# huawei-noah/Speech-Backbones

Hardware: NVIDIA H100
Metric: mel-frames/sec at N=50 reverse-diffusion steps (higher is better)
Workload: dtype f32

## Files before the change

speech-backbones_b200/csrc/sbk_api.cu:

```cuda
#include "sbk_host.h"

#include <math.h>
#include <stdarg.h>
#include <stdio.h>
#include <stdlib.h>
#include <string.h>

#include <algorithm>
#include <map>
#include <string>
#include <vector>

using namespace sbk;

static thread_local char g_err[1024] = "";
int sbk::fail(int code, const char* fmt, ...) {
    va_list ap;
    va_start(ap, fmt);
    vsnprintf(g_err, sizeof(g_err), fmt, ap);
    va_end(ap);
    return code;
}

namespace {
// ... 323 lines not shown
        CU(cudaMemcpy(h->d_freqs, f.data(), half * sizeof(float), cudaMemcpyHostToDevice));
    }
    if (!h->d_zero) {
        CU(cudaMalloc(&h->d_zero, 8192));
        CU(cudaMemset(h->d_zero, 0, 8192));
    }
    free_plan(h);
    h->is_packed = true;
    return SBK_OK;
}

namespace {
struct Bufs {
    float *A[3], *Bf[3], *X[3], *Y[3], *S[3], *D[3], *U1;
    float *kv_part, *ctx, *w_eff, *b_eff;
    std::map<const void*, float*> lo;
};
}

static size_t layout(const sbk_handle* h, int B, int T, int tb_rows, Arena& ar, Bufs* bf, Plan* pl) {
    const sbk_config& c = h->cfg;
    const int dim = c.dim, H = c.n_feats;
    const size_t P[3] = {(size_t)H * T, (size_t)(H / 2) * (T / 2), (size_t)(H / 4) * (T / 4)};
    const int C[3] = {dim, dim * 2, dim * 4};
    auto f = [&](size_t n) { return (float*)ar.take(n * sizeof(float)); };
    const size_t osz = c.precision == SBK_PREC_BF16 ? 2 : 4;
    const bool x3 = c.precision == SBK_PREC_FP32X3;
    Bufs b{};
    auto fo = [&](size_t n) {
        float* r = (float*)ar.take(n * osz);
        if (x3) { float* l = (float*)ar.take(n * osz); if (r) b.lo[r] = l; }
        return r;
    };
    for (int l = 0; l < 3; ++l) {
        const size_t n = (size_t)B * P[l] * C[l];
        b.A[l] = f(n); b.Bf[l] = fo(n); b.X[l] = fo(n); b.Y[l] = fo(n);
        b.S[l] = l > 0 ? fo(n) : nullptr;
        b.D[l] = l > 0 ? fo((size_t)B * P[l] * C[l - 1]) : nullptr;
    }
    b.U1 = fo((size_t)B * P[1] * C[1]);
    const size_t mt0 = (P[0] + attn_kv_tile_pixels() - 1) / attn_kv_tile_pixels();
    b.kv_part = f((size_t)B * mt0 * kHeads * kKvPartFloats);
    b.ctx = f((size_t)B * kHeads * 1024);
    b.w_eff = f((size_t)B * C[2] * C[2] * (x3 ? 2 : 1));
    b.b_eff = f(C[2]);
    if (bf) *bf = b;
    Plan dummy;
    Plan& p = pl ? *pl : dummy;
// ... 48 lines not shown
    auto stats_slot = [&]() { return pl.stats + (size_t)(gn_slot++) * B * kGroups * 2; };
    auto gnref = [&](const double* st, const std::string& blk, int C, int lvl) {
        GnRef g; g.stats = st; g.gamma = h->w.get(blk + ".block.1.weight"); g.beta = h->w.get(blk + ".block.1.bias");
        g.inv_count = 1.0f / ((float)(C / kGroups) * (float)Hs[lvl] * (float)Ws[lvl]);
        return g;
    };
    auto base_ig = [&](int geom, int lvl_in, int lvl_out) {
        IgemmParams p; memset(&p, 0, sizeof(p));
        p.geom = geom; p.B = B; p.T = T;
        p.Hin = Hs[lvl_in]; p.Win = Ws[lvl_in]; p.Hout = Hs[lvl_out]; p.Wout = Ws[lvl_out];
        p.in_lvl = lvl_in; p.out_lvl = lvl_out; p.mask = pl.mask; p.step = pl.step_cur;
        return p;
    };
    const bool use_tc = c.precision != SBK_PREC_FP32;
    const bool x3 = c.precision == SBK_PREC_FP32X3;
    auto LO = [&](const void* q) -> float* { auto it = bf.lo.find(q); return it == bf.lo.end() ? nullptr : it->second; };
    const int num_sms = device_sm_count();
    const char* rows_env = getenv("SBK_CONV3_ROWS");
    const int conv_rows_env = rows_env ? atoi(rows_env) : 0;
    const bool b16 = c.precision == SBK_PREC_BF16;
    const double osz = b16 ? 2.0 : 4.0;
    const int fmt_raw = use_tc ? 1 : 0, fmt_opnd = b16 ? 2 : fmt_raw;
    const int form = b16 ? FORM_BF16 : (x3 ? FORM_X3 : (use_tc ? FORM_TF32 : FORM_NHWC));
    auto push = [&](Op& op, const float* dbg, int64_t numel) {
        op.dbg_ptr = dbg; op.dbg_numel = numel;
        const bool raw_out = op.kind == OP_FIRST || op.kind == OP_CTX || (op.kind == OP_CONVTC && op.tc.geom == G_C3);
        op.dbg_fmt = raw_out ? fmt_raw : fmt_opnd;
        if (op.kind == OP_IGEMM) {
            const IgemmParams& p = op.ig;
            const double cin = p.c0 + p.c1, opx = (double)B * p.Hout * p.Wout, ipx = (double)B * p.Hin * p.Win;
            const double taps = p.geom == G_PW ? 1 : (p.geom == G_UP ? 4 : 9);
// ... 9 lines not shown
            op.bytes = 4.0 * B * H0 * T * (op.fn.C + 3.0);
        }
        pl.ops.push_back(op);
    };
    auto npix = [&](int lvl) { return (int64_t)B * Hs[lvl] * Ws[lvl]; };

    auto tc_conv = [&](const std::string& name, int geom, const std::string& wkey, const std::string& bkey, int lvl,
                       const float* in0, int c0, const float* in1, int c1, int cout, float* out, double* st) {
        Op op; op.name = name; op.kind = OP_CONVTC;
        ConvTcParams& p = op.tc; memset(&p, 0, sizeof(p));
        p.geom = geom; p.in0 = in0; p.c0 = c0; p.in1 = in1; p.c1 = c1; p.H = Hs[lvl]; p.W = Ws[lvl]; p.B = B;
        p.Ho = p.H; p.Wo = p.W;
        p.wpk = h->w.get(wkey); p.bias = bkey.empty() ? nullptr : h->w.get(bkey); p.out = out; p.Cout = cout;
        p.epi = EPI_PLAIN; p.ostats = st; p.mask = pl.mask; p.T = T; p.lvl = lvl; p.zero_page = h->d_zero;
        p.form = form; p.nt = conv_tc_ntile(geom, cout, form);
        if (x3) { p.in0_lo = LO(in0); p.in1_lo = LO(in1); p.out_corr = geom != G_C3 ? LO(out) : nullptr; }
        if (geom == G_C3) {
            const long long wt = (Ws[lvl] + 127) / 128;
            const long long tiles2 = (long long)B * wt * ((Hs[lvl] + 1) / 2) * (cout / 64);
            bool two = tiles2 >= 4LL * num_sms;
            if (conv_rows_env == 1 || conv_rows_env == 2) two = conv_rows_env == 2;
            const bool wide = p.nt == 128;
            if (two && (!wide || h->w.packed.count(wkey + "64"))) {
                p.rows = 2;
                if (wide) { p.nt = 64; p.wpk = h->w.get(wkey + "64"); }
            } else if (wide) {
                const long long tiles = (long long)B * wt * Hs[lvl] * (cout / 128);
                if (tiles * 2 <= num_sms && h->w.packed.count(wkey + "64")) { p.nt = 64; p.wpk = h->w.get(wkey + "64"); }
            }
        }
        const double taps = geom == G_PW ? 1.0 : (geom == G_UP ? 4.0 : 9.0);
// ... 29 lines not shown
            Op op = tc_conv(r.prefix + ".block1.raw", G_C3, r.prefix + ".block1.wtc", r.prefix + ".block1.block.0.bias", lvl,
                            in0, c0, in1, c1, r.cout, A, st1);
            push(op, A, npix(lvl) * r.cout);
        } else {
            ffma_block_conv(r.prefix + ".block1.raw", r.prefix + ".block1.w", r.prefix + ".block1.block.0.bias", lvl,
                            in0, c0, in1, c1, r.cout, A, st1, PRO_MASK, nullptr, k);
        }
        const GnRef g1 = gnref(st1, r.prefix + ".block1", r.cout, lvl);
        float* h2 = Bb;
        if (use_tc) {
            {
                Op op; op.kind = OP_GNACT; op.name = r.prefix + ".block1.act";
                GnActParams& p = op.ga; memset(&p, 0, sizeof(p));
                p.raw = A; p.gn = g1; p.tb = pl.tb + h->tb_off[k]; p.tb_stride = pl.tb_stride; p.step = pl.step_cur;
                p.mask = pl.mask; p.T = T; p.lvl = lvl; p.out = Bb; p.B = B; p.H = Hs[lvl]; p.W = Ws[lvl]; p.C = r.cout;
                p.form = form; p.out_lo = LO(Bb);
                op.bytes = (4.0 + osz) * npix(lvl) * r.cout;
                push(op, nullptr, 0);
            }
            Op op = tc_conv(r.prefix + ".block2.raw", G_C3, r.prefix + ".block2.wtc", r.prefix + ".block2.block.0.bias", lvl,
                            Bb, r.cout, nullptr, 0, r.cout, A, st2);
            push(op, A, npix(lvl) * r.cout);
            h2 = A;
        } else {
            ffma_block_conv(r.prefix + ".block2.raw", r.prefix + ".block2.w", r.prefix + ".block2.block.0.bias", lvl,
                            A, r.cout, nullptr, 0, r.cout, Bb, st2, PRO_GN, &g1, k);
        }
        const GnRef g2 = gnref(st2, r.prefix + ".block2", r.cout, lvl);
        if (k == 0 || r.cin == r.cout) {
            Op op; op.kind = OP_RESFINAL; op.name = r.prefix + ".out";
            ResFinalParams& p = op.rf; memset(&p, 0, sizeof(p));
            p.h2raw = h2; p.gn = g2;
            p.mask = pl.mask; p.T = T; p.lvl = lvl; p.out = out; p.B = B; p.H = Hs[lvl]; p.W = Ws[lvl]; p.C = r.cout;
            p.out_mask = store_masked ? 1 : 0; p.form = form; p.out_lo = LO(out);
            if (k == 0) {
                p.x = nullptr; p.mu = pl.mu; p.xt = pl.xt; p.spk_s = pl.spk_s; p.cin = cin0;
                p.wres = h->w.get(r.prefix + ".res.w"); p.bres = h->w.get(r.prefix + ".res_conv.bias");
                if (vc) { p.r_extra = pl.vc_rextra; p.step = pl.step_cur; }
                pl.first_res_op = (int)pl.ops.size();
            } else {
                p.x = in0;
            }
            op.bytes = (4.0 + (k == 0 ? 0.0 : osz) + osz) * npix(lvl) * r.cout;
            push(op, out, npix(lvl) * r.cout);
        } else if (use_tc) {
            Op op = tc_conv(r.prefix + ".out", G_PW, r.prefix + ".res.wtc", r.prefix + ".res_conv.bias", lvl,
                            in0, c0, in1, c1, r.cout, out, nullptr);
            op.tc.epi = EPI_RES; op.tc.rraw = h2; op.tc.rgn = g2; op.tc.out_mask = store_masked ? 1 : 0;
            op.bytes += 4.0 * npix(lvl) * r.cout;
// ... 3 lines not shown
            op.ig = base_ig(G_PW, lvl, lvl);
            IgemmParams& p = op.ig;
            p.in0 = in0; p.c0 = c0; p.in1 = in1; p.c1 = c1;
            p.w = h->w.get(r.prefix + ".res.w"); p.bias = h->w.get(r.prefix + ".res_conv.bias");
            p.out = out; p.Cout = r.cout; p.pro = PRO_MASK; p.epi = EPI_RES;
            p.rraw = h2; p.rgn = g2;
            push(op, out, npix(lvl) * r.cout);
        }
    };
    auto attention = [&](int k, int lvl, const float* x, float* out) {
        const AttnInfo& a = h->attns[k];
        int mt = igemm_mtiles(G_PW, Hs[lvl], Ws[lvl], Hs[lvl], Ws[lvl]);
        if (use_tc) {
            Op op = tc_conv(a.prefix + ".kvpart", G_PW, a.prefix + ".kv.wtc", "", lvl, x, a.c, nullptr, 0, 256, nullptr, nullptr);
            op.tc.epi = EPI_KV; op.tc.kv_part = bf.kv_part;
            op.bytes = (x3 ? 8.0 : osz) * npix(lvl) * a.c;
            op.flops += 2.0 * npix(lvl) * 4096.0;
            mt = (Hs[lvl] * Ws[lvl] + attn_kv_tile_pixels() - 1) / attn_kv_tile_pixels();
            push(op, nullptr, 0);
        } else {
            Op op; op.kind = OP_IGEMM; op.name = a.prefix + ".kvpart";
            op.ig = base_ig(G_PW, lvl, lvl);
            IgemmParams& p = op.ig;
            p.in0 = x; p.c0 = a.c; p.w = h->w.get(a.prefix + ".kv.w"); p.Cout = 256; p.pro = PRO_NONE; p.epi = EPI_KV;
            p.kv_part = bf.kv_part; p.out = nullptr;
            push(op, nullptr, 0);
        }
        {
            Op op; op.kind = OP_CTX; op.name = a.prefix + ".ctx";
            op.cx.kv_part = bf.kv_part; op.cx.mtiles = mt; op.cx.ctx = bf.ctx; op.cx.B = B;
            push(op, bf.ctx, (int64_t)B * kHeads * 1024);
// ... 674 lines not shown
```

speech-backbones_b200/csrc/sbk_attn_x3.cu:

```cuda
#include "sbk_tc.cuh"

#include <type_traits>

namespace sbk {

using namespace tc;

namespace kx3 {
constexpr int PX = 64;
constexpr int KCH = 8;
constexpr int XS = KCH * PX * 16;
constexpr int WS = 2 * KCH * 128 * 16;
constexpr int STAGE = XS + WS;
constexpr int STAGES = 2;
constexpr int OPI = (PX / 4) * 128 * 16;
constexpr int THREADS = 256 + 32;
constexpr int NBARS = 2 * STAGES;
constexpr size_t SMEM = (size_t)STAGES * STAGE + 4 * OPI + 4 * 128 * 4 + NBARS * 8 + 16;
static_assert(SMEM <= 227 * 1024, "shared memory budget");
}

template <int MODE>
__global__ void __launch_bounds__(kx3::THREADS, 1) k_attn_kv_wg(const ConvTcParams p) {
    using namespace kx3;
    constexpr bool X3 = MODE == 2;
    constexpr int EPC = MODE == 1 ? 8 : 4;
    constexpr int KMAIN = MODE == 1 ? K_BF16 : K_TF32;
    extern __shared__ __align__(1024) uint8_t smem[];
    uint8_t* sS = smem;
    uint8_t* kp = sS + STAGES * STAGE;
    uint8_t* vt = kp + OPI;
    uint8_t* pc = vt + OPI;
    uint8_t* vc = pc + OPI;
    float* s_mx = reinterpret_cast<float*>(vc + OPI);
// ... 13 lines not shown
    if (tid == 0) {
        for (int s = 0; s < STAGES; ++s) { mbar_init(full(s), 1); mbar_init(empty(s), 8); }
        fence_barrier_init();
    }
    __syncthreads();

    if (warp < 8) {
        const int wg = warp >> 2, wt = tid & 127;
        const int row = tid & 127, half = tid >> 7;
        constexpr uint32_t D_HI = desc_hi(128);
        const uint32_t s0 = smem_u32(sS);
        uint32_t it = 0;
        for (int t = blockIdx.x; t < total; t += gridDim.x) {
            const int b = t / items, mt = t - b * items;
            float acc[64];
            for (int ks = 0; ks < ksteps_t; ++ks, ++it) {
                const int s = it % STAGES;
                mbar_wait(full(s), (it / STAGES) & 1);
                const uint32_t xs = s0 + s * STAGE;
                const uint32_t x_lo = desc_lo(xs, PX * 16), w_lo = desc_lo(xs + XS + wg * (KCH * 128 * 16), 128 * 16);
                auto issue = [&](auto kind) {
#pragma unroll
                    for (int kk = 0; kk < KCH / 2; ++kk)
                        wgmma<128, decltype(kind)::value>(acc, desc_pack(x_lo + (uint32_t)(kk * 2 * PX), D_HI),
                                                          desc_pack(w_lo + (uint32_t)(kk * 2 * 128), D_HI), (ks | kk) != 0 ? 1u : 0u);
                };
                wg_fence();
                if (X3 && (ks & 1) == 0) issue(std::integral_constant<int, K_F16>{});
                else issue(std::integral_constant<int, KMAIN>{});
                wg_commit();
                wg_wait<0>();
                wg_fence_regs(acc);
                __syncwarp();
                if (lane == 0) mbar_arrive(empty(s));
            }
            {
                uint8_t* img = wg == 0 ? kp : vt;
#pragma unroll
                for (int i = 0; i < 64; ++i) {
                    const int px = frag_row(wt, i), r = frag_col(wt, i);
                    *reinterpret_cast<float*>(img + ((size_t)(px / 4) * 128 + r) * 16 + (px % 4) * 4) = acc[i];
                }
            }
            asm volatile("bar.sync 1, 256;" ::: "memory");
// ... 73 lines not shown
        }
    } else {
        uint32_t it = 0;
        const int chs = p.c0 / EPC;
        for (int t = blockIdx.x; t < total; t += gridDim.x) {
            const int b = t / items, mt = t - b * items;
            const int m0 = mt * PX, m_hi = m0 + PX < HW ? m0 + PX : HW;
            const int hh0 = m0 / p.W, ww0 = m0 - hh0 * p.W;
            for (int ks = 0; ks < ksteps_t; ++ks, ++it) {
                const int s = it % STAGES;
                const int kb = X3 ? ks >> 1 : ks;
                const bool corr = X3 && (ks & 1) == 0;
                const uint32_t xs = smem_u32(sS) + s * STAGE;
                if (lane == 0) {
                    mbar_wait(empty(s), ((it / STAGES) & 1) ^ 1);
                    mbar_arrive_expect_tx(full(s), STAGE);
                    bulk_g2s(xs + XS, reinterpret_cast<const uint8_t*>(p.wpk) + (size_t)(X3 ? 2 * kb + (corr ? 1 : 0) : ks) * WS, WS, full(s));
                }
                __syncwarp();
                if (lane < KCH) {
                    const uint8_t* src = reinterpret_cast<const uint8_t*>(corr ? p.in0_lo : p.in0);
                    const int k = lane, cl = kb * KCH + k;
                    int m = m0, hh = hh0, ww = ww0, qx = 0;
                    while (m < m_hi) {
                        const int n = (p.W - ww) < (m_hi - m) ? (p.W - ww) : (m_hi - m);
                        bulk_g2s(xs + (k * PX + qx) * 16, src + (((long long)(b * p.H + hh) * chs + cl) * p.W + ww) * 16,
                                 (uint32_t)n * 16u, full(s));
                        m += n; qx += n; ++hh; ww = 0;
                    }
                    if (qx < PX) bulk_g2s(xs + (k * PX + qx) * 16, p.zero_page, (uint32_t)(PX - qx) * 16u, full(s));
                }
            }
        }
    }
}

// ... 19 lines not shown
```

speech-backbones_b200/csrc/sbk_conv_tc.cu:

```cuda
#include "sbk_tc.cuh"

#include <cuda_fp16.h>
#include <string.h>
#include <type_traits>

namespace sbk {

namespace tc {

constexpr int TPX = 128;
constexpr int NCONS = 256;
constexpr int NTHREADS = NCONS + 128;
constexpr int PROD_REGS = 40, CONS_REGS = 232;
static_assert(128 * PROD_REGS + NCONS * CONS_REGS <= 65536, "register file");

template <int GEOM, int R = 1> struct Geo;
template <int R> struct Geo<G_C3, R> {
    static_assert(R == 1 || R == 2, "3x3 tiles are 1 or 2 rows");
    static constexpr int ROWS = R, HR = R + 2, PXP = TPX + 2, TAPS = 9, KCH = 2, NACC = R;
};
template <> struct Geo<G_PW> { static constexpr int ROWS = 1, HR = 1, PXP = TPX, TAPS = 1, KCH = 8, NACC = 1; };
template <> struct Geo<G_DOWN> { static constexpr int ROWS = 1, HR = 3, PXP = 2 * (TPX + 1), TAPS = 9, KCH = 2, NACC = 1; };
template <> struct Geo<G_UP> { static constexpr int ROWS = 1, HR = 3, PXP = TPX + 2, TAPS = 16, KCH = 2, NACC = 4; };

template <int K> struct GeoC1 { static constexpr int ROWS = 1, HR = 1, PXP = TPX + 64, TAPS = K, KCH = 2, NACC = 1; };
template <> struct Geo<G_C1K3> : GeoC1<3> {};
template <> struct Geo<G_C1K7> : GeoC1<7> {};
// ... 7 lines not shown

using namespace tc;


template <int GEOM, int NT, int R = 1> struct Depth {
    using G = Geo<GEOM, R>;
    static constexpr int STAGE_BYTES = G::KCH * G::HR * G::PXP * 16 + G::TAPS * G::KCH * NT * 16;
    static constexpr int LDS = NT + 4;
    static constexpr int SD_BYTES = TPX * LDS * 4;
    static constexpr int FIT = (220 * 1024 - SD_BYTES) / STAGE_BYTES;
    static constexpr int STAGES = FIT > 6 ? 6 : FIT;
    static constexpr size_t SMEM = (size_t)STAGES * STAGE_BYTES + SD_BYTES + 3 * STAGES * 8 + 128 * 4 * G::ROWS + 3 * NT * 4 + 64;
    static_assert(STAGES >= 2, "need at least 2 stages");
    static_assert(SMEM <= 227 * 1024, "shared memory budget");
};

template <int GEOM, bool BF16, int NT, bool RES, bool X3, bool VOC = false, int R = 1>
__device__ __forceinline__ void conv_tc_body(const ConvTcParams& p) {
    static_assert(!(X3 && BF16), "fp32x3 runs on tf32 operands");
    using G = Geo<GEOM, R>;
    using D = Depth<GEOM, NT, R>;
    constexpr int NACC = G::NACC, ROWS = G::ROWS;
    constexpr bool ROW2 = ROWS == 2;
    constexpr bool CHUNKED = X3 && GEOM != G_UP;
    const int FLUSH = CHUNKED ? 6 : (1 << 30);
    constexpr int STAGES = D::STAGES, LDS = D::LDS;
    constexpr int LAG = STAGES >= 3 ? STAGES - 2 : 0;
    constexpr int HR = G::HR, PXP = G::PXP, TAPS = G::TAPS, KCH = G::KCH;
    constexpr int EPC = BF16 ? 8 : 4;
    constexpr int CPS = KCH * EPC;
// ... 9 lines not shown
    constexpr int KMAIN = BF16 ? K_BF16 : K_TF32;

    extern __shared__ __align__(1024) uint8_t smem[];
    uint8_t* sA = smem;
    uint8_t* sB = sA + STAGES * A_STAGE_BYTES;
    float* sD = reinterpret_cast<float*>(sB + STAGES * B_STAGE_BYTES);
    uint64_t* bars = reinterpret_cast<uint64_t*>(sD + TPX * LDS);
    float* s_st = reinterpret_cast<float*>(bars + 3 * STAGES);
    float* s_rg = s_st + 128 * ROWS;

    const int tid = threadIdx.x, warp = __shfl_sync(0xffffffffu, tid >> 5, 0), lane = tid & 31;
    const int Cin = p.c0 + p.c1;
    const int HW = p.H * p.W;
    const int ksteps = Cin / CPS * conv_tc_stage_rows(GEOM);
    const int ksteps_t = X3 ? 2 * ksteps : ksteps;
    const int wt_w = (GEOM == G_DOWN ? p.Wo : p.W), wt_h = (GEOM == G_DOWN ? p.Ho : p.H);
    const int wtiles = (wt_w + SPAN - 1) / SPAN;
    const int mtiles = GEOM == G_PW ? (HW + TPX - 1) / TPX : wtiles * ((wt_h + ROWS - 1) / ROWS);
    const int ntn = p.Cout / NT;
    const int total_tiles = p.B * mtiles * ntn;
    auto decode = [&](int t, int& b, int& h0, int& w0, int& n0) {
        const int nt = t % ntn; const int r = t / ntn;
        const int mt = r % mtiles; b = r / mtiles; n0 = nt * NT;
        if (GEOM == G_PW) { w0 = 0; h0 = mt; }
        else { w0 = (mt % wtiles) * SPAN; h0 = (mt / wtiles) * ROWS; }
    };

    const uint32_t bar0 = smem_u32(bars);
    auto full_b = [&](int s) { return bar0 + 8u * s; };
    auto empty = [&](int s) { return bar0 + 8u * (STAGES + s); };
    auto full_a = [&](int s) { return bar0 + 8u * (2 * STAGES + s); };

    if (tid == 0) {
        for (int s = 0; s < STAGES; ++s) { mbar_init(full_a(s), NCONS / 32); mbar_init(full_b(s), 1); mbar_init(empty(s), NCONS / 32); }
        fence_barrier_init();
    }
    if (tid < 128 * ROWS) s_st[tid] = 0.f;
    __syncthreads();

    if (warp < NCONS / 32) {
        setmaxnreg_inc<CONS_REGS>();
        const int wg = warp >> 2, wt = tid & 127;
        uint32_t it = 0;
        constexpr int SLOTS = HR * PXP * KCH;
        constexpr int PER = BULK ? 1 : (SLOTS + NCONS - 1) / NCONS;
        uint32_t sl_dst[PER]; long long sl_off[PER]; int sl_chunk[PER]; bool sl_ok[PER];
        const uint32_t a0 = smem_u32(sA), b0 = smem_u32(sB);
        constexpr uint32_t D_HI = desc_hi(128);
        float acc[NACC][FR];
// ... 15 lines not shown
                    sl_off[j] = (ok ? (long long)(b * p.H + hi) : 0) * 1048576 + (ok ? wi : 0);
                    sl_dst[j] = in ? (uint32_t)(k * PLANE + (r * PXP + q) * 16) : 0xFFFFFFFFu;
                }
            }
            auto produce = [&](int ks) {
                const uint32_t g = it + ks;
                const int s = g % STAGES;
                mbar_wait(empty(s), ((g / STAGES) & 1) ^ 1);
                const int kb = X3 ? ks / 2 : ks;
                const bool lo = X3 && (ks & 1) == 0;
                const int ck = kb * KCH;
                const bool second = ck * EPC >= p.c0;
                const uint8_t* src = reinterpret_cast<const uint8_t*>(second ? (lo ? p.in1_lo : p.in1) : (lo ? p.in0_lo : p.in0));
                const int chs = (second ? p.c1 : p.c0) / EPC;
                const int c0k = second ? ck - p.c0 / EPC : ck;
#pragma unroll
                for (int j = 0; j < PER; ++j) {
                    if (sl_dst[j] == 0xFFFFFFFFu) continue;
                    const long long row = sl_off[j] / 1048576, wi = sl_off[j] % 1048576;
                    const uint8_t* gp = src + ((row * chs + c0k + sl_chunk[j]) * p.W + wi) * 16;
                    cp_async16(a0 + s * A_STAGE_BYTES + sl_dst[j], gp, sl_ok[j] ? 16u : 0u);
                }
            };
            auto release = [&](uint32_t g) {
                __syncwarp();
                if (lane == 0) mbar_arrive(empty(g % STAGES));
            };
            auto wait_full = [&](uint32_t g) {
                const int s = g % STAGES;
                const uint32_t ph = (g / STAGES) & 1;
                if (!BULK) mbar_wait(full_a(s), ph);
                mbar_wait(full_b(s), ph);
            };
            auto issue = [&](uint32_t g, bool first, auto kind) {
                constexpr int KD = decltype(kind)::value;
                const int s = g % STAGES;
                const uint32_t a_lo = desc_lo(a0 + s * A_STAGE_BYTES, PLANE) + (uint32_t)(ROW2 ? wg * PXP : 64 * wg);
                const uint32_t b_lo = desc_lo(b0 + s * B_STAGE_BYTES, NT * 16);
                const uint32_t dil = C1 ? (uint32_t)p.dil : 0u;
                wg_fence();
#pragma unroll
                for (int kk = 0; kk < KCH / 2; ++kk) {
                    const uint32_t a_k = a_lo + (uint32_t)(kk * 2 * (PLANE / 16)), b_k = b_lo + (uint32_t)(kk * 2 * NT);
                    if (GEOM == G_UP) {
#pragma unroll
                        for (int phase = 0; phase < 4; ++phase) {
// ... 21 lines not shown
                                              desc_pack(b_k + (uint32_t)(tap * KCH * NT), D_HI), (!first || (kk | tap) != 0) ? 1u : 0u);
                        }
                    }
                }
                wg_commit();
            };
            auto fence_acc = [&]() {
#pragma unroll
                for (int a = 0; a < NACC; ++a) wg_fence_regs(acc[a]);
            };
            constexpr auto kind_c = std::integral_constant<int, K_F16>{};
            constexpr auto kind_m = std::integral_constant<int, KMAIN>{};
            if constexpr (BULK && X3) {
                auto step = [&](int ks, bool first, auto kind) {
                    const uint32_t g = it + ks;
                    wait_full(g);
                    issue(g, first, kind);
                    wg_wait<1>();
                    __syncwarp();
                    if (lane == 0 && !first) mbar_arrive(empty((g - 1) % STAGES));
                };
                if constexpr (CHUNKED) {
#pragma unroll
                    for (int a = 0; a < NACC; ++a)
#pragma unroll
                        for (int i = 0; i < FR; ++i) acc[a][i] = 0.f;
                }
                bool first_run = true;
                for (int ks = 0; ks < ksteps_t;) {
                    const int run_hi = ksteps_t - ks < FLUSH ? ksteps_t : ks + FLUSH;
                    bool first = true;
// ... 32 lines not shown
                    if constexpr (CHUNKED) {
                        const bool first = run_lo == 0, last = ks == ksteps_t - 1 || ks - run_lo == FLUSH - 1;
#pragma unroll
                        for (int a = 0; a < NACC; ++a)
#pragma unroll
                            for (int i = 0; i < FR; ++i) sum[a][i] = last ? (first ? acc[a][i] : sum[a][i] + acc[a][i]) : sum[a][i];
                    }
                };
                if constexpr (BULK) {
                    for (int ks = 0; ks < ksteps_t; ++ks) compute(ks, kind_m);
                } else {
                    for (int ks = 0; ks < ksteps_t + LAG; ++ks) {
                        if (ks < ksteps_t) produce(ks);
                        cp_async_commit();
                        if (ks >= LAG) {
                            cp_async_wait<LAG>();
                            fence_proxy_async();
                            __syncwarp();
                            if (lane == 0) mbar_arrive(full_a((it + ks - LAG) % STAGES));
                            if (X3 && ((ks - LAG) & 1) == 0) compute(ks - LAG, kind_c);
                            else compute(ks - LAG, kind_m);
                        }
                    }
                }
            }
            it += ksteps_t;

            if constexpr (RES) {
                asm volatile("bar.sync 1, 256;" ::: "memory");
                const int cpg = p.Cout / kGroups;
                for (int i = tid; i < NT; i += NCONS) {
                    const int c = n0 + i, g = c / cpg;
                    const double sm_ = p.rgn.stats[(b * kGroups + g) * 2], ss = p.rgn.stats[(b * kGroups + g) * 2 + 1];
                    const double m = sm_ * (double)p.rgn.inv_count;
                    double var = ss * (double)p.rgn.inv_count - m * m;
// ... 201 lines not shown
                const int gb = n0 / cpg, ng = (NT + cpg - 1) / cpg;
                const int r = tid / (ng * 2), e = tid - r * (ng * 2);
                if (tid < ng * 2 * ROWS) {
                    double tot = 0.0;
                    float* sl = s_st + r * 128 + e;
#pragma unroll
                    for (int w8 = 0; w8 < NCONS / 32; ++w8) { tot += (double)sl[w8 * 16]; sl[w8 * 16] = 0.f; }
                    if (!ROW2 || h0 + r < Ho)
                        atomicAdd(&p.ostats[((long long)b * kGroups + gb + (e >> 1)) * 2 + (e & 1)], tot);
                }
                asm volatile("bar.sync 1, 256;" ::: "memory");
            }
        }
    } else {
        setmaxnreg_dec<PROD_REGS>();
        if (warp != NCONS / 32) return;
        uint32_t it = 0;
        const float* zero = p.zero_page;
        uint32_t stage_pat[STAGES];
#pragma unroll
        for (int i = 0; i < STAGES; ++i) stage_pat[i] = 0xFFFFFFFFu;
        for (int t = blockIdx.x; t < total_tiles; t += gridDim.x) {
            int b, h0, w0, n0;
            decode(t, b, h0, w0, n0);
            const uint8_t* wsrc = reinterpret_cast<const uint8_t*>(p.wpk) + (size_t)b * p.w_bstride_bytes +
                                  (size_t)(n0 / NT) * ksteps * (X3 ? 2 : 1) * B_STAGE_BYTES;
            constexpr int PADK = GEOM == G_C7 ? 3 : 1;
            for (int ks = 0; ks < ksteps_t; ++ks, ++it) {
                const int s = it % STAGES;
                const int st = X3 ? ks / 2 : ks, var = X3 ? (ks & 1) : 1;
                const int kb = st / conv_tc_stage_rows(GEOM), krow = st - kb * conv_tc_stage_rows(GEOM);
                if (lane == 0) {
                    mbar_wait(empty(s), ((it / STAGES) & 1) ^ 1);
                    uint32_t a_tx = BULK ? A_STAGE_BYTES : 0;
                    if (BULK && GEOM != G_PW) {
                        const int pad = C1 ? p.pad : PADK;
                        const int wlo = w0 - pad < 0 ? 0 : w0 - pad, whi = w0 + SPAN + pad > p.W ? p.W : w0 + SPAN + pad;
                        const int qlo = wlo - (w0 - pad), qhi = qlo + (whi - wlo);
                        const uint32_t pat = (uint32_t)qlo | ((uint32_t)qhi << 16);
                        if (stage_pat[s] != pat) {
                            stage_pat[s] = pat;
                            if (qlo > 0 || qhi < PXP) {
                                uint8_t* st = sA + s * A_STAGE_BYTES;
                                for (int k = 0; k < KCH; ++k)
                                    for (int r = 0; r < HR; ++r) {
                                        uint4* rowp = reinterpret_cast<uint4*>(st + k * PLANE + (r * PXP) * 16);
                                        for (int q = 0; q < qlo; ++q) rowp[q] = make_uint4(0u, 0u, 0u, 0u);
                                        for (int q = qhi; q < PXP; ++q) rowp[q] = make_uint4(0u, 0u, 0u, 0u);
                                    }
                                fence_proxy_async();
                            }
                        }
                        int vrows = 0;
                        for (int r = 0; r < HR; ++r) { const int hi = C1 ? 0 : h0 - PADK + krow + r; vrows += (hi >= 0 && hi < p.H) ? 1 : 0; }
                        a_tx -= (uint32_t)(KCH * vrows * (PXP - (qhi - qlo))) * 16u;
                    }
                    mbar_arrive_expect_tx(full_b(s), B_STAGE_BYTES + a_tx);
                    bulk_g2s(smem_u32(sB + s * B_STAGE_BYTES), wsrc + (size_t)(X3 ? 2 * st + (var == 0) : ks) * B_STAGE_BYTES,
                             B_STAGE_BYTES, full_b(s));
                }
                __syncwarp();
                if (BULK && lane < KCH * HR) {
                    const uint32_t a_s = smem_u32(sA) + s * A_STAGE_BYTES;
                    const int k = lane / HR, r = lane - k * HR;
                    const int ck = kb * KCH + k;
                    const bool second = ck * EPC >= p.c0;
                    const uint8_t* src = reinterpret_cast<const uint8_t*>(var == 0 ? (second ? p.in1_lo : p.in0_lo) : (second ? p.in1 : p.in0));
                    const int chs = (second ? p.c1 : p.c0) / EPC;
                    const int cl = second ? ck - p.c0 / EPC : ck;
                    if (GEOM == G_PW) {
                        long long m = (long long)(h0 + r) * TPX;
                        const long long m_hi = m >= HW ? m : (m + TPX < HW ? m + TPX : HW);
                        int q = 0;
                        if (m < m_hi) {
                            int hh = (int)(m / p.W), ww = (int)(m - (long long)hh * p.W);
                            while (m < m_hi) {
                                const int n = (int)((p.W - ww) < (m_hi - m) ? (p.W - ww) : (m_hi - m));
// ... 61 lines not shown
int conv_tc_ntile(int geom, int Cout, int form) {
    if (geom == G_UP || geom == G_DOWN) return 64;
    if (geom_is_c1(geom)) return Cout % 128 == 0 && form != FORM_X3 ? 128 : (Cout % 64 == 0 ? 64 : 32);
    if (geom == G_C7 && form == FORM_X3) return 64;
    return Cout % 128 == 0 ? 128 : 64;
}

static constexpr int tc_key(int geom, int form, int nt, int rows = 1, bool res = false, bool voc = false) {
    return ((((geom * 4 + form) * 256 + nt) * 2 + rows - 1) * 2 + (res ? 1 : 0)) * 2 + (voc ? 1 : 0);
}

int launch_conv_tc(const ConvTcParams& p, cudaStream_t s) {
    if (p.form < FORM_TF32 || p.form > FORM_BF16 || p.nt <= 0 || p.nt > 128 || p.Cout % p.nt != 0) return -1;
    if (p.geom == G_PW && p.epi == EPI_KV) return launch_attn_kv(p, s);
    if (geom_is_c1(p.geom) && (p.dil < 1 || p.pad < 0 || 2 * p.pad > 64)) return -1;
    const int rows = p.geom == G_C3 && p.rows == 2 ? 2 : 1;
    const bool res = p.geom == G_PW && p.epi == EPI_RES;
    const bool voc = p.voc && p.geom == G_PW && p.form == FORM_BF16;
    constexpr int T = FORM_TF32, X = FORM_X3, B = FORM_BF16;
    switch (tc_key(p.geom, p.form, p.nt, rows, res, voc)) {
        case tc_key(G_C3, T, 128):                  return launch_tc<G_C3, T, 128>(p, s);
        case tc_key(G_C3, T, 64):                   return launch_tc<G_C3, T, 64>(p, s);
        case tc_key(G_C3, T, 64, 2):                return launch_tc<G_C3, T, 64, false, 2>(p, s);
        case tc_key(G_C3, B, 128):                  return launch_tc<G_C3, B, 128>(p, s);
        case tc_key(G_C3, B, 64):                   return launch_tc<G_C3, B, 64>(p, s);
        case tc_key(G_C3, B, 64, 2):                return launch_tc<G_C3, B, 64, false, 2>(p, s);
        case tc_key(G_C3, X, 128):                  return launch_tc<G_C3, X, 128>(p, s);
        case tc_key(G_C3, X, 64):                   return launch_tc<G_C3, X, 64>(p, s);
        case tc_key(G_C3, X, 64, 2):                return launch_tc<G_C3, X, 64, false, 2>(p, s);
        case tc_key(G_PW, T, 128):                  return launch_tc<G_PW, T, 128>(p, s);
// ... 109 lines not shown
```

speech-backbones_b200/csrc/sbk_kernels.cu:

```cuda
#include "sbk_internal.h"

#include <math.h>
#include <type_traits>

namespace sbk {


__device__ __forceinline__ float mish_f(float x) {
    float n = expf(fminf(x, 20.f));
    float a = n * (n + 2.f);
    float r = a / (a + 2.f);
    return x > 20.f ? x : x * r;
}

__device__ __forceinline__ float mish_fast_f(float x) {
    const float n = __expf(fminf(x, 20.f));
    const float a = n * (n + 2.f);
    return x > 20.f ? x : x * __fdividef(a, a + 2.f);
}

__device__ __forceinline__ float mish_rt(float x, int exact) { return exact ? mish_f(x) : mish_fast_f(x); }
template <bool EXACT> __device__ __forceinline__ float mish_sel(float x) { return EXACT ? mish_f(x) : mish_fast_f(x); }

__device__ __forceinline__ void gn_mean_rstd(const GnRef& g, int b, int grp, float& mean, float& rstd) {
// ... 617 lines not shown
                    if (p.out_mask) { o.x *= mk; o.y *= mk; o.z *= mk; o.w *= mk; }
                } else if (mk != 0.f) {
                    float4 a;
                    if constexpr (TAIL == TAIL_ACT) a = pt; else a = opnd_f32(xv[u]);
                    o.x = mish_sel<X3>((r[u].x - pm.x) * ps.x + pb.x) + a.x;
                    o.y = mish_sel<X3>((r[u].y - pm.y) * ps.y + pb.y) + a.y;
                    o.z = mish_sel<X3>((r[u].z - pm.z) * ps.z + pb.z) + a.z;
                    o.w = mish_sel<X3>((r[u].w - pm.w) * ps.w + pb.w) + a.w;
                    if constexpr (FORM == FORM_TF32 && TAIL == TAIL_ACT) o = make_float4(rna_tf32(o.x), rna_tf32(o.y), rna_tf32(o.z), rna_tf32(o.w));
                }
                const long long oi = obase + (long long)(h0 + u) * ohs + w * LPF;
                if constexpr (B16) {
                    reinterpret_cast<uint2*>(p.out)[oi] = make_uint2(pack_bf16x2_f(o.x, o.y), pack_bf16x2_f(o.z, o.w));
                } else {
                    reinterpret_cast<float4*>(p.out)[oi] = o;
                    if constexpr (X3) reinterpret_cast<float4*>(p.out_lo)[oi] = corr_chunk(o.x, o.y, o.z, o.w);
                }
            }
        }
    }
}

template <int FORM>
__global__ void __launch_bounds__(256) k_gn_act(const GnActParams p) { planar_ew<FORM, TAIL_ACT>(p, p.raw); }

template <int FORM, bool PLANAR>
__global__ void __launch_bounds__(256, FORM == FORM_BF16 ? (PLANAR ? 2 : 4) : 0) k_resfinal(const ResFinalParams p) {
    planar_ew<FORM, PLANAR ? TAIL_PLANAR : TAIL_ID>(p, p.h2raw);
}

int launch_gn_act(const GnActParams& p, cudaStream_t s) {
// ... 575 lines not shown
```

Before: 13000.

## Compute fp32x3 correction operands in shared memory instead of global lo buffers

Removes the separate global low-part (correction) activation buffers in FP32X3 mode. The correction operand is now derived in shared memory from the already-loaded main stage, by dedicated converter warps in the bulk conv path, by consumer warps in the cp.async path, and inline in the attention KV kernel. This avoids writing and re-reading a second full activation tensor per layer, at the cost of extra shared-memory conversion work and added barrier and phase logic. It only matters when precision is FP32X3; other precisions are unaffected.

Result: faster. 13460, median of 6 (+3.6%).

```diff
diff --git a/speech-backbones_b200/csrc/sbk_api.cu b/speech-backbones_b200/csrc/sbk_api.cu
--- a/speech-backbones_b200/csrc/sbk_api.cu
+++ b/speech-backbones_b200/csrc/sbk_api.cu
@@ -361,7 +361,6 @@
 struct Bufs {
     float *A[3], *Bf[3], *X[3], *Y[3], *S[3], *D[3], *U1;
     float *kv_part, *ctx, *w_eff, *b_eff;
-    std::map<const void*, float*> lo;
 };
 }
 
@@ -374,11 +373,7 @@
     const size_t osz = c.precision == SBK_PREC_BF16 ? 2 : 4;
     const bool x3 = c.precision == SBK_PREC_FP32X3;
     Bufs b{};
-    auto fo = [&](size_t n) {
-        float* r = (float*)ar.take(n * osz);
-        if (x3) { float* l = (float*)ar.take(n * osz); if (r) b.lo[r] = l; }
-        return r;
-    };
+    auto fo = [&](size_t n) { return (float*)ar.take(n * osz); };
     for (int l = 0; l < 3; ++l) {
         const size_t n = (size_t)B * P[l] * C[l];
         b.A[l] = f(n); b.Bf[l] = fo(n); b.X[l] = fo(n); b.Y[l] = fo(n);
@@ -457,7 +452,6 @@
     };
     const bool use_tc = c.precision != SBK_PREC_FP32;
     const bool x3 = c.precision == SBK_PREC_FP32X3;
-    auto LO = [&](const void* q) -> float* { auto it = bf.lo.find(q); return it == bf.lo.end() ? nullptr : it->second; };
     const int num_sms = device_sm_count();
     const char* rows_env = getenv("SBK_CONV3_ROWS");
     const int conv_rows_env = rows_env ? atoi(rows_env) : 0;
@@ -497,7 +491,6 @@
         p.wpk = h->w.get(wkey); p.bias = bkey.empty() ? nullptr : h->w.get(bkey); p.out = out; p.Cout = cout;
         p.epi = EPI_PLAIN; p.ostats = st; p.mask = pl.mask; p.T = T; p.lvl = lvl; p.zero_page = h->d_zero;
         p.form = form; p.nt = conv_tc_ntile(geom, cout, form);
-        if (x3) { p.in0_lo = LO(in0); p.in1_lo = LO(in1); p.out_corr = geom != G_C3 ? LO(out) : nullptr; }
         if (geom == G_C3) {
             const long long wt = (Ws[lvl] + 127) / 128;
             const long long tiles2 = (long long)B * wt * ((Hs[lvl] + 1) / 2) * (cout / 64);
@@ -557,7 +550,7 @@
                 GnActParams& p = op.ga; memset(&p, 0, sizeof(p));
                 p.raw = A; p.gn = g1; p.tb = pl.tb + h->tb_off[k]; p.tb_stride = pl.tb_stride; p.step = pl.step_cur;
                 p.mask = pl.mask; p.T = T; p.lvl = lvl; p.out = Bb; p.B = B; p.H = Hs[lvl]; p.W = Ws[lvl]; p.C = r.cout;
-                p.form = form; p.out_lo = LO(Bb);
+                p.form = form;
                 op.bytes = (4.0 + osz) * npix(lvl) * r.cout;
                 push(op, nullptr, 0);
             }
@@ -575,7 +568,7 @@
             ResFinalParams& p = op.rf; memset(&p, 0, sizeof(p));
             p.h2raw = h2; p.gn = g2;
             p.mask = pl.mask; p.T = T; p.lvl = lvl; p.out = out; p.B = B; p.H = Hs[lvl]; p.W = Ws[lvl]; p.C = r.cout;
-            p.out_mask = store_masked ? 1 : 0; p.form = form; p.out_lo = LO(out);
+            p.out_mask = store_masked ? 1 : 0; p.form = form;
             if (k == 0) {
                 p.x = nullptr; p.mu = pl.mu; p.xt = pl.xt; p.spk_s = pl.spk_s; p.cin = cin0;
                 p.wres = h->w.get(r.prefix + ".res.w"); p.bres = h->w.get(r.prefix + ".res_conv.bias");
@@ -609,7 +602,7 @@
         if (use_tc) {
             Op op = tc_conv(a.prefix + ".kvpart", G_PW, a.prefix + ".kv.wtc", "", lvl, x, a.c, nullptr, 0, 256, nullptr, nullptr);
             op.tc.epi = EPI_KV; op.tc.kv_part = bf.kv_part;
-            op.bytes = (x3 ? 8.0 : osz) * npix(lvl) * a.c;
+            op.bytes = osz * npix(lvl) * a.c;
             op.flops += 2.0 * npix(lvl) * 4096.0;
             mt = (Hs[lvl] * Ws[lvl] + attn_kv_tile_pixels() - 1) / attn_kv_tile_pixels();
             push(op, nullptr, 0);
diff --git a/speech-backbones_b200/csrc/sbk_attn_x3.cu b/speech-backbones_b200/csrc/sbk_attn_x3.cu
--- a/speech-backbones_b200/csrc/sbk_attn_x3.cu
+++ b/speech-backbones_b200/csrc/sbk_attn_x3.cu
@@ -18,6 +18,7 @@
 constexpr int NBARS = 2 * STAGES;
 constexpr size_t SMEM = (size_t)STAGES * STAGE + 4 * OPI + 4 * 128 * 4 + NBARS * 8 + 16;
 static_assert(SMEM <= 227 * 1024, "shared memory budget");
+static_assert(XS <= OPI && STAGES == 2, "fp32x3: the converted x fits a context image; a K stage is the whole ring");
 }
 
 template <int MODE>
@@ -61,6 +62,40 @@
         for (int t = blockIdx.x; t < total; t += gridDim.x) {
             const int b = t / items, mt = t - b * items;
             float acc[64];
+            if constexpr (X3) {
+                for (int kb = 0; kb < ksteps; ++kb, it += 2) {
+                    const int sc = it % STAGES, sm = (it + 1) % STAGES;
+                    mbar_wait(full(sc), (it / STAGES) & 1);
+                    mbar_wait(full(sm), ((it + 1) / STAGES) & 1);
+                    const uint32_t xc = s0 + sc * STAGE, xm = s0 + sm * STAGE;
+                    uint8_t* cx = (kb & 1) ? vc : pc;
+                    {
+                        const float4* src = reinterpret_cast<const float4*>(sS + sm * STAGE);
+#pragma unroll
+                        for (int i = tid; i < XS / 16; i += 256) {
+                            const float4 v = src[i];
+                            reinterpret_cast<float4*>(cx)[i] = corr_chunk(v.x, v.y, v.z, v.w);
+                        }
+                    }
+                    fence_proxy_async();
+                    asm volatile("bar.sync 1, 256;" ::: "memory");
+                    const uint32_t c_lo = desc_lo(smem_u32(cx), PX * 16), x_lo = desc_lo(xm, PX * 16);
+                    const uint32_t wc_lo = desc_lo(xc + XS + wg * (KCH * 128 * 16), 128 * 16), wm_lo = desc_lo(xm + XS + wg * (KCH * 128 * 16), 128 * 16);
+                    wg_fence();
+#pragma unroll
+                    for (int kk = 0; kk < KCH / 2; ++kk)
+                        wgmma<128, K_F16>(acc, desc_pack(c_lo + (uint32_t)(kk * 2 * PX), D_HI), desc_pack(wc_lo + (uint32_t)(kk * 2 * 128), D_HI),
+                                          (kb | kk) != 0 ? 1u : 0u);
+#pragma unroll
+                    for (int kk = 0; kk < KCH / 2; ++kk)
+                        wgmma<128, K_TF32>(acc, desc_pack(x_lo + (uint32_t)(kk * 2 * PX), D_HI), desc_pack(wm_lo + (uint32_t)(kk * 2 * 128), D_HI), 1u);
+                    wg_commit();
+                    wg_wait<0>();
+                    wg_fence_regs(acc);
+                    __syncwarp();
+                    if (lane == 0) { mbar_arrive(empty(sc)); mbar_arrive(empty(sm)); }
+                }
+            } else
             for (int ks = 0; ks < ksteps_t; ++ks, ++it) {
                 const int s = it % STAGES;
                 mbar_wait(full(s), (it / STAGES) & 1);
@@ -73,8 +108,7 @@
                                                           desc_pack(w_lo + (uint32_t)(kk * 2 * 128), D_HI), (ks | kk) != 0 ? 1u : 0u);
                 };
                 wg_fence();
-                if (X3 && (ks & 1) == 0) issue(std::integral_constant<int, K_F16>{});
-                else issue(std::integral_constant<int, KMAIN>{});
+                issue(std::integral_constant<int, KMAIN>{});
                 wg_commit();
                 wg_wait<0>();
                 wg_fence_regs(acc);
@@ -178,12 +212,12 @@
                 const uint32_t xs = smem_u32(sS) + s * STAGE;
                 if (lane == 0) {
                     mbar_wait(empty(s), ((it / STAGES) & 1) ^ 1);
-                    mbar_arrive_expect_tx(full(s), STAGE);
+                    mbar_arrive_expect_tx(full(s), corr ? WS : STAGE);
                     bulk_g2s(xs + XS, reinterpret_cast<const uint8_t*>(p.wpk) + (size_t)(X3 ? 2 * kb + (corr ? 1 : 0) : ks) * WS, WS, full(s));
                 }
                 __syncwarp();
-                if (lane < KCH) {
-                    const uint8_t* src = reinterpret_cast<const uint8_t*>(corr ? p.in0_lo : p.in0);
+                if (lane < KCH && !corr) {
+                    const uint8_t* src = reinterpret_cast<const uint8_t*>(p.in0);
                     const int k = lane, cl = kb * KCH + k;
                     int m = m0, hh = hh0, ww = ww0, qx = 0;
                     while (m < m_hi) {
diff --git a/speech-backbones_b200/csrc/sbk_conv_tc.cu b/speech-backbones_b200/csrc/sbk_conv_tc.cu
--- a/speech-backbones_b200/csrc/sbk_conv_tc.cu
+++ b/speech-backbones_b200/csrc/sbk_conv_tc.cu
@@ -11,6 +11,7 @@
 constexpr int TPX = 128;
 constexpr int NCONS = 256;
 constexpr int NTHREADS = NCONS + 128;
+constexpr int NCONV = 96;
 constexpr int PROD_REGS = 40, CONS_REGS = 232;
 static_assert(128 * PROD_REGS + NCONS * CONS_REGS <= 65536, "register file");
 
@@ -48,6 +49,7 @@
     static_assert(STAGES >= 2, "need at least 2 stages");
     static_assert(SMEM <= 227 * 1024, "shared memory budget");
 };
+template <int GEOM, int NT, int R> constexpr bool x3_depth_ok = Depth<GEOM, NT, R>::STAGES >= 3;
 
 template <int GEOM, bool BF16, int NT, bool RES, bool X3, bool VOC = false, int R = 1>
 __device__ __forceinline__ void conv_tc_body(const ConvTcParams& p) {
@@ -87,6 +89,8 @@
     const int HW = p.H * p.W;
     const int ksteps = Cin / CPS * conv_tc_stage_rows(GEOM);
     const int ksteps_t = X3 ? 2 * ksteps : ksteps;
+    const bool insm = X3 && p.in0_lo == nullptr;
+    static_assert(!X3 || x3_depth_ok<GEOM, NT, R>, "in-SM correction operand: stage g needs stage g + 1, three stages");
     const int wt_w = (GEOM == G_DOWN ? p.Wo : p.W), wt_h = (GEOM == G_DOWN ? p.Ho : p.H);
     const int wtiles = (wt_w + SPAN - 1) / SPAN;
     const int mtiles = GEOM == G_PW ? (HW + TPX - 1) / TPX : wtiles * ((wt_h + ROWS - 1) / ROWS);
@@ -105,7 +109,8 @@
     auto full_a = [&](int s) { return bar0 + 8u * (2 * STAGES + s); };
 
     if (tid == 0) {
-        for (int s = 0; s < STAGES; ++s) { mbar_init(full_a(s), NCONS / 32); mbar_init(full_b(s), 1); mbar_init(empty(s), NCONS / 32); }
+        constexpr int A_WARPS = X3 && BULK ? NCONV / 32 : NCONS / 32;
+        for (int s = 0; s < STAGES; ++s) { mbar_init(full_a(s), A_WARPS); mbar_init(full_b(s), 1); mbar_init(empty(s), NCONS / 32); }
         fence_barrier_init();
     }
     if (tid < 128 * ROWS) s_st[tid] = 0.f;
@@ -151,6 +156,7 @@
                 const uint8_t* src = reinterpret_cast<const uint8_t*>(second ? (lo ? p.in1_lo : p.in1) : (lo ? p.in0_lo : p.in0));
                 const int chs = (second ? p.c1 : p.c0) / EPC;
                 const int c0k = second ? ck - p.c0 / EPC : ck;
+                if (X3 && insm && lo) return;
 #pragma unroll
                 for (int j = 0; j < PER; ++j) {
                     if (sl_dst[j] == 0xFFFFFFFFu) continue;
@@ -163,10 +169,11 @@
                 __syncwarp();
                 if (lane == 0) mbar_arrive(empty(g % STAGES));
             };
-            auto wait_full = [&](uint32_t g) {
+            auto wait_full = [&](uint32_t g, bool conv = false) {
                 const int s = g % STAGES;
                 const uint32_t ph = (g / STAGES) & 1;
                 if (!BULK) mbar_wait(full_a(s), ph);
+                else if (conv) mbar_wait(full_a(s), (g / (STAGES % 2 ? 2 * STAGES : STAGES)) & 1);
                 mbar_wait(full_b(s), ph);
             };
             auto issue = [&](uint32_t g, bool first, auto kind) {
@@ -218,7 +225,7 @@
             if constexpr (BULK && X3) {
                 auto step = [&](int ks, bool first, auto kind) {
                     const uint32_t g = it + ks;
-                    wait_full(g);
+                    wait_full(g, insm && decltype(kind)::value == K_F16);
                     issue(g, first, kind);
                     wg_wait<1>();
                     __syncwarp();
@@ -281,11 +288,23 @@
                         if (ks < ksteps_t) produce(ks);
                         cp_async_commit();
                         if (ks >= LAG) {
+                            const bool corr = X3 && ((ks - LAG) & 1) == 0;
+                            if (X3 && insm && corr) {
+                                static_assert(!X3 || LAG >= 1, "the main gather runs ahead of its correction sub-stage");
+                                cp_async_wait<(LAG > 0 ? LAG - 1 : 0)>();
+                                const uint32_t sc = (it + ks - LAG) % STAGES, sm = (it + ks - LAG + 1) % STAGES;
+#pragma unroll
+                                for (int j = 0; j < PER; ++j) {
+                                    if (sl_dst[j] == 0xFFFFFFFFu) continue;
+                                    const float4 v = *reinterpret_cast<const float4*>(sA + sm * A_STAGE_BYTES + sl_dst[j]);
+                                    *reinterpret_cast<float4*>(sA + sc * A_STAGE_BYTES + sl_dst[j]) = corr_chunk(v.x, v.y, v.z, v.w);
+                                }
+                            }
                             cp_async_wait<LAG>();
                             fence_proxy_async();
                             __syncwarp();
                             if (lane == 0) mbar_arrive(full_a((it + ks - LAG) % STAGES));
-                            if (X3 && ((ks - LAG) & 1) == 0) compute(ks - LAG, kind_c);
+                            if (corr) compute(ks - LAG, kind_c);
                             else compute(ks - LAG, kind_m);
                         }
                     }
@@ -517,7 +536,36 @@
         }
     } else {
         setmaxnreg_dec<PROD_REGS>();
-        if (warp != NCONS / 32) return;
+        if (warp != NCONS / 32) {
+            if constexpr (X3 && BULK) {
+                if (insm) {
+                    const int ct = tid - (NCONS + 32);
+                    uint32_t it = 0;
+                    for (int t = blockIdx.x; t < total_tiles; t += gridDim.x) {
+                        for (int ks = 0; ks < ksteps_t; ks += 2, it += 2) {
+                            const uint32_t sc = it % STAGES, sm = (it + 1) % STAGES;
+                            mbar_wait(full_b(sm), ((it + 1) / STAGES) & 1);
+                            const float4* src = reinterpret_cast<const float4*>(sA + sm * A_STAGE_BYTES);
+                            float4* dst = reinterpret_cast<float4*>(sA + sc * A_STAGE_BYTES);
+                            constexpr int NCHK = A_STAGE_BYTES / 16, UN = 4;
+                            for (int i0 = ct; i0 < NCHK; i0 += UN * NCONV) {
+                                float4 v[UN];
+#pragma unroll
+                                for (int u = 0; u < UN; ++u)
+                                    if (i0 + u * NCONV < NCHK) v[u] = src[i0 + u * NCONV];
+#pragma unroll
+                                for (int u = 0; u < UN; ++u)
+                                    if (i0 + u * NCONV < NCHK) dst[i0 + u * NCONV] = corr_chunk(v[u].x, v[u].y, v[u].z, v[u].w);
+                            }
+                            fence_proxy_async();
+                            __syncwarp();
+                            if (lane == 0) mbar_arrive(full_a(sc));
+                        }
+                    }
+                }
+            }
+            return;
+        }
         uint32_t it = 0;
         const float* zero = p.zero_page;
         uint32_t stage_pat[STAGES];
@@ -533,15 +581,18 @@
                 const int s = it % STAGES;
                 const int st = X3 ? ks / 2 : ks, var = X3 ? (ks & 1) : 1;
                 const int kb = st / conv_tc_stage_rows(GEOM), krow = st - kb * conv_tc_stage_rows(GEOM);
+                const bool conv = X3 && BULK && insm && var == 0;
                 if (lane == 0) {
                     mbar_wait(empty(s), ((it / STAGES) & 1) ^ 1);
-                    uint32_t a_tx = BULK ? A_STAGE_BYTES : 0;
+                    uint32_t a_tx = BULK && !conv ? A_STAGE_BYTES : 0;
                     if (BULK && GEOM != G_PW) {
                         const int pad = C1 ? p.pad : PADK;
                         const int wlo = w0 - pad < 0 ? 0 : w0 - pad, whi = w0 + SPAN + pad > p.W ? p.W : w0 + SPAN + pad;
                         const int qlo = wlo - (w0 - pad), qhi = qlo + (whi - wlo);
                         const uint32_t pat = (uint32_t)qlo | ((uint32_t)qhi << 16);
-                        if (stage_pat[s] != pat) {
+                        if (conv) {
+                            stage_pat[s] = pat;
+                        } else if (stage_pat[s] != pat) {
                             stage_pat[s] = pat;
                             if (qlo > 0 || qhi < PXP) {
                                 uint8_t* st = sA + s * A_STAGE_BYTES;
@@ -556,14 +607,14 @@
                         }
                         int vrows = 0;
                         for (int r = 0; r < HR; ++r) { const int hi = C1 ? 0 : h0 - PADK + krow + r; vrows += (hi >= 0 && hi < p.H) ? 1 : 0; }
-                        a_tx -= (uint32_t)(KCH * vrows * (PXP - (qhi - qlo))) * 16u;
+                        if (!conv) a_tx -= (uint32_t)(KCH * vrows * (PXP - (qhi - qlo))) * 16u;
                     }
                     mbar_arrive_expect_tx(full_b(s), B_STAGE_BYTES + a_tx);
                     bulk_g2s(smem_u32(sB + s * B_STAGE_BYTES), wsrc + (size_t)(X3 ? 2 * st + (var == 0) : ks) * B_STAGE_BYTES,
                              B_STAGE_BYTES, full_b(s));
                 }
                 __syncwarp();
-                if (BULK && lane < KCH * HR) {
+                if (BULK && !conv && lane < KCH * HR) {
                     const uint32_t a_s = smem_u32(sA) + s * A_STAGE_BYTES;
                     const int k = lane / HR, r = lane - k * HR;
                     const int ck = kb * KCH + k;
@@ -655,6 +706,7 @@
     if (p.form < FORM_TF32 || p.form > FORM_BF16 || p.nt <= 0 || p.nt > 128 || p.Cout % p.nt != 0) return -1;
     if (p.geom == G_PW && p.epi == EPI_KV) return launch_attn_kv(p, s);
     if (geom_is_c1(p.geom) && (p.dil < 1 || p.pad < 0 || 2 * p.pad > 64)) return -1;
+    if (p.form == FORM_X3 && p.c1 > 0 && (p.in0_lo == nullptr) != (p.in1_lo == nullptr)) return -1;
     const int rows = p.geom == G_C3 && p.rows == 2 ? 2 : 1;
     const bool res = p.geom == G_PW && p.epi == EPI_RES;
     const bool voc = p.voc && p.geom == G_PW && p.form == FORM_BF16;
diff --git a/speech-backbones_b200/csrc/sbk_kernels.cu b/speech-backbones_b200/csrc/sbk_kernels.cu
--- a/speech-backbones_b200/csrc/sbk_kernels.cu
+++ b/speech-backbones_b200/csrc/sbk_kernels.cu
@@ -655,7 +655,9 @@
                     reinterpret_cast<uint2*>(p.out)[oi] = make_uint2(pack_bf16x2_f(o.x, o.y), pack_bf16x2_f(o.z, o.w));
                 } else {
                     reinterpret_cast<float4*>(p.out)[oi] = o;
-                    if constexpr (X3) reinterpret_cast<float4*>(p.out_lo)[oi] = corr_chunk(o.x, o.y, o.z, o.w);
+                    if constexpr (X3) {
+                        if (p.out_lo) reinterpret_cast<float4*>(p.out_lo)[oi] = corr_chunk(o.x, o.y, o.z, o.w);
+                    }
                 }
             }
         }
```
